# QizhiPei/FABind

Measured on AMD Instinct MI355X. Metric: complexes/sec fwd+bwd (1500p/40l nodes), full IaBNet on the whole graph (pocket model + 4-layer complex model + distance-map head on all nodes / pairs) with the pocket-cls + pocket-centre + coord + distmap + distmap-by-coords + distill losses (BASELINE configs[2] read literally), higher is better.
Workload: dtype bf16

## Files before the change

### fabind_amd/_lib.py

```python
import ctypes
import os

import torch

from . import config as _cfg

_HERE = os.path.dirname(os.path.abspath(__file__))
LIB_PATH = _cfg.knob("FABIND_LIB") or os.path.join(_HERE, "libfabind_hip.so")

ABI_VERSION = 19
DT_F32, DT_BF16 = 0, 1
ACT_NONE, ACT_SILU, ACT_RELU, ACT_SIGMOID, ACT_STORED_DERIV = 0, 1, 2, 3, 4
GEMM_FAM_NT_F32, GEMM_FAM_NT_F32_BF16, GEMM_FAM_NT_BF16, GEMM_FAM_GLDS, GEMM_FAM_PIPE, GEMM_FAM_X3, GEMM_FAM_X3_PRO, GEMM_FAM_PERSIST = range(8)

_vp, _i, _f, _l = ctypes.c_void_p, ctypes.c_int, ctypes.c_float, ctypes.c_long


class GemmArgs(ctypes.Structure):
    _fields_ = [(n, _vp) for n in ("A", "A2", "W", "C", "bias", "R", "r_index", "dotvec", "dot_out", "aux", "groups", "C2")] + \
               [(n, _i) for n in ("M", "N", "K", "K1", "lda", "lda2", "ldw", "ldc", "ldr", "ldaux", "dot_ld",
                                  "a_dtype", "w_dtype", "c_dtype", "aux_dtype", "act_pro", "act_epi", "dact_epi",
                                  "accumulate", "store_preact", "n_groups", "max_m", "max_n", "groups_ext", "epi_fast", "k_splits")] + \
               [("alpha", _f), ("p_drop", _f), ("drop_seed", ctypes.c_uint)] + \
               [(n, _vp) for n in ("row_mu", "row_rs", "col_c", "C16")] + [("ldc16", _i), ("split3", _i), ("r_dtype", _i), ("c2_bf16", _i)]
# ... 105 lines not shown
    "fabind_rowdot_bwd": [_vp, _i, _vp, _i, _vp, _i, _i, _i, _vp, _vp, _vp, _i, _vp],
    "fabind_edge_geom_bwd": [_vp, _vp, _vp, _vp, _vp, _vp, _vp, _vp, _vp, _vp, _i, _i, _i, _vp, _vp, _vp, _vp],
    "fabind_gcl_pre_bwd": [_vp, _i, _i, _vp, _vp, _i, _vp, _vp, _vp, _i, _vp],
    "fabind_gather_dact": [_vp, _i, _vp, _vp, _i, _i, _vp, _i, _i, _i, _vp],
    "fabind_coord_update_bwd": [_vp, _vp, _vp, _i, _i, _f, _vp, _vp, _vp, _vp],
    "fabind_cross_attn_bwd": [_vp, _i, _vp, _i, _vp, _i, _i, _i, _vp, _i, _i, _i, _f, _vp, _vp, _vp, _vp, _vp, _vp, _vp,
                              _vp, _vp, _vp],
    "fabind_pair_bias_cat": [_vp, _i, _vp, _i, _i, _i, _vp, _i, _vp, _i, _vp, _vp, _i, _vp, _i, _vp, _vp],
    "fabind_batched_transpose_pad": [_vp, _i, _vp, _i, _i, _i, _i, _vp, _vp],
    "fabind_node_chain_fwd": [_vp, _i, _vp, _i, _vp, _vp, _vp, _vp, _vp, _vp, _i, _i, _vp, _i, _vp, _i, _vp, _i, _i, _i, _vp],
    "fabind_node_chain_x3_fwd": [_vp, _i, _vp, _i, _vp, _vp, _vp, _vp, _vp, _vp, _vp, _vp, _vp, _vp, _i, _i, _vp, _i, _vp, _i, _vp, _i, _vp, _i, _vp, _i,
                                 _i, _i, _vp],
    "fabind_rows_hadamard_bwd": [_vp, _i, _i, _vp, _i, _i, _vp, _vp, _vp, _i, _vp, _i, _vp],
    "fabind_pair_hadamard_bwd_grid": [_vp, _i, _i, _vp, _i, _i, _vp, _vp, _vp, _vp, _i, _vp, _i, _vp],
    "fabind_pair_hadamard_bwd_rows": [_vp, _i, _i, _vp, _i, _i, _vp, _i, _i, _vp, _vp, _vp, _vp, _i, _vp, _i, _vp, _i, _vp],
    "fabind_pair_hadamard_bwd": [_vp, _i, _i, _vp, _vp, _i, _i, _vp, _vp, _i, _i, _vp, _vp, _i, _vp, _vp, _i, _vp, _vp, _i,
                                 _vp],
    "fabind_inter_attn_bwd": [_vp, _i, _vp, _i, _i, _vp, _vp, _vp, _vp, _vp, _vp, _vp, _vp, _vp, _vp, _vp, _vp, _f, _i,
                              _vp, _vp, _vp, _vp, _vp, _vp, _vp, _vp, _vp, _vp, _i, _vp],
    "fabind_inter_attn_bwd_rows": [_vp, _i, _vp, _i, _i, _vp, _vp, _vp, _vp, _vp, _vp, _vp, _vp, _vp, _vp, _vp, _vp, _f, _i,
                                   _vp, _vp, _vp, _vp, _vp, _vp, _vp, _vp, _vp, _vp, _i, _vp, _i, _i, _vp],
    "fabind_las_step_bwd": [_vp, _vp, _vp, _vp, _vp, _vp, _vp, _vp, _i, _i, _f, _f, _vp, _vp, _vp],
    "fabind_pair_bias_bwd": [_vp, _i, _vp, _i, _i, _vp, _vp, _i, _i, _i, _vp, _vp, _vp, _vp, _vp],
    "fabind_pair_bias_btcat": [_vp, _i, _vp, _vp, _vp, _i, _i, _i, _vp, _i, _i, _vp],
    "fabind_pair_bias_finish": [_vp, _vp, _i, _i, _vp, _vp, _i, _vp, _vp, _l, _vp],
    "fabind_pack_frag_multi": [_vp, _vp, _i, _vp],
    "fabind_lower_bound": [_vp, _i, _vp, _i, _vp, _vp],
    "fabind_pocket_center_fwd": [_vp, _vp, _vp, _vp, _i, _i, _f, _i, _vp, _vp, _vp],
    "fabind_pocket_center_bwd": [_vp, _vp, _vp, _vp, _i, _i, _f, _vp, _vp, _vp, _vp, _vp],
    "fabind_pair_dist_fwd": [_vp, _i, _i, _vp, _vp, _f, _f, _f, _vp, _vp],
    "fabind_pair_dist_bwd": [_vp, _i, _i, _vp, _vp, _vp, _f, _f, _f, _vp, _vp, _vp],
    "fabind_block_hadamard_fwd": [_vp, _i, _i, _vp, _i, _vp, _i, _i, _vp, _i, _vp],
    "fabind_block_hadamard_bwd": [_vp, _i, _i, _vp, _i, _vp, _i, _vp, _i, _i, _vp, _i, _i, _vp, _vp, _i, _vp, _i, _vp],
    "fabind_loss_fwd": [_vp, _vp, _l, _vp, _vp, _vp, _l, _vp, _vp, _i, _vp, _l, _vp, _vp, _l, _f, _f, _f, _f, _f, _f, _vp, _vp, _vp, _vp, _vp, _vp],
    "fabind_loss_bwd": [_vp, _vp, _l, _vp, _vp, _vp, _l, _vp, _vp, _i, _l, _vp, _vp, _l, _f, _f, _f, _f, _f, _f, _vp, _vp, _vp,
                        _vp, _vp, _vp, _vp, _vp, _vp],
    "fabind_layernorm_fwd": [_vp, _vp, _vp, _f, _i, _i, _vp, _vp, _vp, _vp],
    "fabind_layernorm_bwd": [_vp, _vp, _vp, _vp, _vp, _i, _i, _vp, _vp, _vp, _vp],
}

_lib = None


def load():
    global _lib
    if _lib is not None:
        return _lib
    if not os.path.exists(LIB_PATH):
        raise RuntimeError(
            "fabind_amd: %s is missing -- build it with `python -m fabind_amd.build` (hipcc, gfx950). "
            "There is no CPU/eager fallback for the hot path." % LIB_PATH)
    lib = ctypes.CDLL(LIB_PATH)
    lib.fabind_last_error.restype = ctypes.c_char_p
    lib.fabind_abi_version.restype = ctypes.c_int
    got = lib.fabind_abi_version()
    if got != ABI_VERSION:
        raise RuntimeError("fabind_amd: %s has ABI version %d, this binding needs %d -- rebuild with `python -m fabind_amd.build`"
                           % (LIB_PATH, got, ABI_VERSION))
    lib.fabind_sizeof_args.argtypes, lib.fabind_sizeof_args.restype = [ctypes.c_int], ctypes.c_int
    lib.fabind_cross_attn_bwd_scratch.argtypes, lib.fabind_cross_attn_bwd_scratch.restype = [_i, _i, _i], ctypes.c_long
    lib.fabind_pair_bias_cat_parts.argtypes, lib.fabind_pair_bias_cat_parts.restype = [_i, _i], ctypes.c_long
    lib.fabind_cross_attn_fused_bwd_scratch.argtypes, lib.fabind_cross_attn_fused_bwd_scratch.restype = [_i, _i, _i, _i, _i], ctypes.c_long
    lib.fabind_cross_attn_fused_bwd_parts.argtypes, lib.fabind_cross_attn_fused_bwd_parts.restype = [_i, _i], ctypes.c_int
    lib.fabind_pair_bias_finish_parts.argtypes, lib.fabind_pair_bias_finish_parts.restype = [_i], ctypes.c_int
    lib.fabind_loss_blocks.argtypes, lib.fabind_loss_blocks.restype = [_l, _l, _l], ctypes.c_int
    for nm in ("fabind_pair_block_tile", "fabind_pair_block_chunk"):
# ... 58 lines not shown
```

### fabind_amd/build.py

```python
import os
import subprocess
import sys

HERE = os.path.dirname(os.path.abspath(__file__))
CSRC = os.path.join(HERE, "csrc")
INCLUDE = os.path.join(os.path.dirname(HERE), "include")
LIB = os.path.join(HERE, "libfabind_hip.so")
SOURCES = ["capi.hip", "gemm.hip", "graph.hip", "gcl.hip", "fused_edge.hip", "fused_edge_fwd2.hip", "fused_edge_fwd3.hip", "fused_edge_bwd3.hip", "fused_edge_bwd4.hip", "pair_fused.hip", "attn.hip", "inter_attn_rows.hip", "attn_mfma.hip", "norm.hip", "bwd.hip", "post_optim.hip", "node_chain.hip", "heads.hip", "symmetry.hip", "optim.hip", "ranking.hip"]
HIPCC = os.environ.get("HIPCC", "/opt/rocm/bin/hipcc")
FLAGS = ["--offload-arch=gfx950", "-O3", "-std=c++17", "-fPIC", "-Wno-comment", "-I" + INCLUDE, "-I" + CSRC]


def _stale(out, deps):
    if not os.path.exists(out):
        return True
    t = os.path.getmtime(out)
    return any(os.path.getmtime(d) > t for d in deps)


def build(force=False, verbose=True):
    objs = []
    hdrs = [os.path.join(CSRC, "common.h"), os.path.join(CSRC, "fused_common.h"), os.path.join(INCLUDE, "fabind_hip.h")]
    procs = []
    for src in SOURCES:
        sp = os.path.join(CSRC, src)
        if not os.path.exists(sp):
            raise RuntimeError("fabind_amd.build: source %s is missing" % sp)
        obj = os.path.join(CSRC, src.replace(".hip", ".o"))
        objs.append(obj)
        if force or _stale(obj, [sp] + hdrs):
            cmd = [HIPCC] + FLAGS + ["-c", sp, "-o", obj]
            if verbose:
                print(" ".join(cmd), flush=True)
            procs.append((src, subprocess.Popen(cmd)))
    for src, p in procs:
        if p.wait() != 0:
            raise RuntimeError("hipcc failed on " + src)
    if force or procs or _stale(LIB, objs):
        cmd = [HIPCC, "--offload-arch=gfx950", "-shared", "-fPIC", "-o", LIB] + objs
        if verbose:
            print(" ".join(cmd), flush=True)
# ... 7 lines not shown
```

### fabind_amd/models/model.py

```python
import random

import torch
import torch.nn as nn
import torch.nn.functional as F
from torch.nn import Linear

from .. import kernels as K
from .. import ops
from ..utils.utils import get_keepNode_tensor, gumbel_softmax_no_random
from .att_model import EfficientMCAttModel


class Transition_diff_out_dim(nn.Module):

    def __init__(self, embedding_channels=256, out_channels=256, n=4):
        super().__init__()
        self.layernorm = nn.LayerNorm(embedding_channels)
        self.linear1 = Linear(embedding_channels, n * embedding_channels)
        self.linear2 = Linear(n * embedding_channels, out_channels)
        torch.nn.init.xavier_uniform_(self.linear1.weight, gain=0.001)
        torch.nn.init.xavier_uniform_(self.linear2.weight, gain=0.001)

    def forward(self, z):
        shp = z.shape
# ... 252 lines not shown
        start = _offsets(reps)
        j = torch.arange(pi.shape[0], device=dev) - start[pi]
        ci = _offsets(ncnt)[pocket_batch][pi] + j
        kn = torch.stack([kcnt, ncnt]).tolist()
        return _Pairs(pi, ci, ops.PairBlocks(kn[0], kn[1], dev))

    def _complex_and_heads(self, data, g, plan=None):
        scale = self.coordinate_scale
        cb = data['compound'].batch
        if plan:
            Xn, Xl, cidx, pidx = plan['Xn'], plan['Xl'], plan['cidx'], plan['pidx']
        else:
            Xn = self.normalize_coord(g['X'].unsqueeze(-2)).float()
            Xl = self.normalize_coord(g['XL'].unsqueeze(-2)).float()
            seg1 = g['segment'].bool() if not g['segment'].is_floating_point() else g['segment'] > 0.5
            cidx = torch.nonzero(~seg1 & ~g['is_global']).squeeze(1)
            pidx = torch.nonzero(seg1 & ~g['is_global']).squeeze(1)
        Xo, Ho = self.complex_model(Xn, g['H'], batch_id=g['batch'], segment_id=g['segment'], mask=g['mask'],
                                    is_global=g['is_global'], compound_edge_index=g['c2c'], LAS_edge_index=g['LAS'],
                                    batched_complex_coord_LAS=Xl, LAS_mask=None)
        coords_n = ops.take_unique_rows(Xo, cidx).squeeze(-2)
        return Ho, cidx, pidx, coords_n

    def _dist_heads(self, data, g, Ho, cidx, pidx, coords_n):
        cb = data['compound'].batch
        pairs = g.get('pairs')
        if pairs is None:
            B = int(cb[-1].item()) + 1
            pairs = self._pair_lists(g['pocket_batch'], cb, torch.bincount(g['pocket_batch'], minlength=B), torch.bincount(cb, minlength=B))
        pi, ci = pairs
        ln = ops.layernorm(ops.take_unique_rows(Ho, torch.cat([pidx, cidx])), self.layernorm.weight, self.layernorm.bias, self.layernorm.eps)
        npk = pidx.shape[0]
        blocks = getattr(pairs, 'blocks', None)
        hd = ops.rows_hadamard(ln, pi, npk + ci, a_sorted=True, blocks=blocks, n_a=npk)
        wd = ops.mm_dtype()
        part = ops.linear_rowdot(hd, self.distmap_mlp[0].weight.to(wd), self.distmap_mlp[0].bias,
                                 self.distmap_mlp[2].weight[0].contiguous(), act_epi=K.ACT_RELU)
        y_pred = (part.sum(1) + self.distmap_mlp[2].bias).sigmoid() * 10
        xp = self.normalize_coord(g['pocket_xyz']).float()
        if blocks is not None and coords_n.is_cuda:
            y_by = ops.pair_dist(xp, coords_n, blocks, scale=self.coordinate_scale, lo=0.0, hi=10.0)
        else:
            y_by = self.unnormalize_coord((xp[pi] - ops.take_rows_few(coords_n, ci)).norm(dim=-1)).clamp(0, 10)
        return y_pred, y_by

    def forward(self, data, stage=1, train=False, plan=None):
        cb = data['compound'].batch
        if plan is not None:
            self._adopt_plan(plan, cb.device)
        if plan is not None:
            keep_idx = plan['keep_idx']
        else:
            keep_idx = torch.nonzero(data['pocket'].keepNode).squeeze(1) if (stage == 1 or self.pocket_pred_model.training) else None
        head = self._pocket_head(data, plan)
        training = self.pocket_pred_model.training
        center = self._soft_center(head['logits'], head['mask'], head['xyz'], noise=training)
        pocket_cls = torch.zeros_like(head['mask'], dtype=data.pocket_idx.dtype)
        pocket_cls[head['pb'], head['loc']] = data.pocket_idx
        if training:
            dist = torch.norm(data.coords_center - center, p=2, dim=-1).mean(dim=-1)
            final_stage = 2 if (dist < self.args.center_dist_threshold and random.random() < self.stage_prob) else 1
        else:
            final_stage = stage
        if final_stage == 2:
            c2 = center
            if self.args.local_eval or (self.args.train_pred_pocket_noise and train):
                c2 = center + self.args.train_pred_pocket_noise * (2 * torch.rand_like(center) - 1)
            g = self._stage2(data, head, c2)
        else:
            cx = data['complex']
            pemb = ops.take_unique_rows(head['p_out'], keep_idx if keep_idx is not None else torch.nonzero(data['pocket'].keepNode).squeeze(1))
# ... 62 lines not shown
```

### fabind_amd/ops.py

```python
import ctypes

import numpy as np
import torch

from . import config as _cfg
from . import kernels as K
from ._lib import GemmArgs, check, dt_code, load, ptr, stream


def act_dtype():
    return torch.float32 if _cfg.fp32_storage() else torch.bfloat16


mm_dtype = act_dtype


def needs_grad(*ts):
    return torch.is_grad_enabled() and any(torch.is_tensor(t) and t.requires_grad for t in ts)


_needs_grad = needs_grad


def _nchunk(rows):
# ... 1755 lines not shown


def six_term_loss(coords, y_pred, y_by, logits, center, coords_true, dis_map, pocket_cls, p_mask, center_true, w):
    f = lambda t: t.float().contiguous()
    cls = pocket_cls.contiguous()
    if cls.dtype not in _CLS_DT:
        cls = cls.float()
    m8 = p_mask.contiguous().view(torch.uint8) if p_mask.dtype == torch.bool else p_mask.to(torch.uint8).contiguous()
    w = {k: float(v) for k, v in w.items()}
    loss, terms = _SixTermLoss.apply(f(coords), f(y_pred), f(y_by), f(logits), f(center), f(coords_true), f(dis_map), cls, m8,
                                     f(center_true), w)
    tt = terms.unbind(0)
    return loss, {n: tt[i] for i, n in enumerate(LOSS_TERM_NAMES)}


_PAIRBLOCK = np.dtype([("pair_off", np.int64), ("P", np.int32), ("C", np.int32), ("p_row0", np.int32), ("c_row0", np.int32),
                       ("tile0", np.int32), ("pad", np.int32)])


class PairBlocks:

    def __init__(self, kcnt, ncnt, dev):
        from .param_pack import _upload
        kc, nc = np.asarray(kcnt, dtype=np.int64), np.asarray(ncnt, dtype=np.int64)
        B = kc.shape[0]
        tp, ch = load().fabind_pair_block_tile(), load().fabind_pair_block_chunk()
        tiles = (kc + tp - 1) // tp
        d = np.zeros(B, dtype=_PAIRBLOCK)
        d["pair_off"] = np.cumsum(kc * nc) - kc * nc
        d["P"], d["C"] = kc, nc
        d["p_row0"], d["c_row0"] = np.cumsum(kc) - kc, np.cumsum(nc) - nc
        d["tile0"] = np.cumsum(tiles) - tiles
        self.B, self.n_tiles, self.n_pairs = int(B), int(tiles.sum()), int((kc * nc).sum())
        self.max_C, self.n_prows, self.n_crows = int(nc.max()) if B else 0, int(kc.sum()), int(nc.sum())
        self.nchunk_max = (self.max_C + ch - 1) // ch
        self.chunk = ch
        row_b = np.repeat(np.arange(B, dtype=np.int32), nc)
        raw = np.concatenate([d.view(np.uint8), row_b.view(np.uint8)]) if B else np.zeros(0, dtype=np.uint8)
        self.buf = _upload(raw, dev) if raw.shape[0] else None
        self.desc_bytes = d.view(np.uint8).shape[0]

    def tensors(self):
        return [self.buf] if self.buf is not None else []

    @property
    def desc_ptr(self):
        return self.buf.data_ptr()

    @property
    def row_b_ptr(self):
        return self.buf.data_ptr() + self.desc_bytes


class _PairDist(torch.autograd.Function):
    @staticmethod
    def forward(ctx, xp, xc, blocks, scale, lo, hi):
        y = torch.empty(blocks.n_pairs, dtype=torch.float32, device=xc.device)
        check(load().fabind_pair_dist_fwd(blocks.desc_ptr, blocks.B, blocks.n_tiles, ptr(xp), ptr(xc), scale, lo, hi, ptr(y), stream()),
              "fabind_pair_dist_fwd")
        ctx.save_for_backward(xp, xc)
        ctx.blocks, ctx.k = blocks, (scale, lo, hi)
        return y

    @staticmethod
    def backward(ctx, dy):
        xp, xc = ctx.saved_tensors
        bl = ctx.blocks
        part = torch.empty((bl.B, 8, bl.max_C, 3), dtype=torch.float32, device=xc.device)
        dxc = torch.empty_like(xc)
        check(load().fabind_pair_dist_bwd(bl.desc_ptr, bl.B, bl.max_C, ptr(xp), ptr(xc), ptr(dy.contiguous().float()), ctx.k[0], ctx.k[1],
                                          ctx.k[2], ptr(part), ptr(dxc), stream()), "fabind_pair_dist_bwd")
        return None, dxc, None, None, None, None


def pair_dist(xp, xc, blocks, scale=1.0, lo=0.0, hi=10.0):
    assert not xp.requires_grad, "pair_dist: the pocket coordinates are data"
    xp, xc = xp.float().contiguous(), xc.float().contiguous()
    assert xp.shape[0] == blocks.n_prows and xc.shape[0] == blocks.n_crows
    return _PairDist.apply(xp, xc, blocks, float(scale), float(lo), float(hi))


RANK_MODES = {"logsigmoid": 0, "dynamic_hinge": 1}
RANK_MAX_GROUP = 1024
COUNT_NAMES = ("ranked_right", "pairs", "hit", "confidence_correct")
# ... 74 lines not shown
```

### include/fabind_hip.h

```cpp
#ifndef FABIND_HIP_H
#define FABIND_HIP_H

#include <stdint.h>

#ifdef __cplusplus
extern "C" {
#endif

#ifndef __HIP_PLATFORM_AMD__
typedef struct ihipStream_t* hipStream_t;
#endif

const char* fabind_last_error(void);
#define FABIND_ABI_VERSION 19
int fabind_abi_version(void);
int fabind_sizeof_args(int which);

typedef struct FabindGemmArgs {
    const void* A;
    const void* A2;
    const void* W;
    void* C;
    const float* bias;
    const void* R;
// ... 243 lines not shown
int fabind_las_step(const float* x, const float* x0, const int* las_i, const int* las_j, const int* las_off,
                    const int* node_off, const int* c_cnt, int B, int max_n, float step, float clampv, float* x_out,
                    unsigned char* pass_mask, hipStream_t stream);

int fabind_pocket_center_fwd(const float* logits, const uint8_t* mask, const float* xyz, const float* noise, int B, int L,
                             float tau, int hard, float* center, float* wsum, hipStream_t stream);
int fabind_pocket_center_bwd(const float* logits, const uint8_t* mask, const float* xyz, const float* noise, int B, int L,
                             float tau, const float* center, const float* wsum, const float* dcenter, float* dlogits,
                             hipStream_t stream);

int fabind_loss_blocks(long n_pair, long n_coord, long n_cls);
int fabind_loss_fwd(const float* coords, const float* coords_true, long n_coord, const float* y_pred, const float* y_by,
                    const float* dis_map, long n_pair, const float* logits, const void* cls, int cls_dt, const uint8_t* mask,
                    long n_cls, const float* center, const float* center_true, long n_center, float w_coord, float w_pair,
                    float w_distill, float w_cls, float w_center, float delta, float* part, unsigned* ticket, float* out,
                    float* loss_out, float* terms_out, hipStream_t stream);
int fabind_loss_bwd(const float* coords, const float* coords_true, long n_coord, const float* y_pred, const float* y_by,
                    const float* dis_map, long n_pair, const float* logits, const void* cls, int cls_dt, long n_cls,
                    const float* center, const float* center_true, long n_center, float w_coord, float w_pair, float w_distill,
                    float w_cls, float w_center, float delta, const float* fwd_out, const float* g_loss, const float* g_terms,
                    float* d_coords, float* d_y_pred, float* d_y_by, float* d_logits, float* d_center, hipStream_t stream);

int fabind_pair_block_tile(void);
int fabind_pair_block_chunk(void);
int fabind_pair_dist_fwd(const void* desc, int B, int n_tiles, const float* xp, const float* xc, float scale, float lo, float hi,
                         float* y, hipStream_t stream);
int fabind_pair_dist_bwd(const void* desc, int B, int max_C, const float* xp, const float* xc, const float* dy, float scale, float lo,
                         float hi, float* part, float* dxc, hipStream_t stream);
int fabind_block_hadamard_fwd(const void* desc, int B, int n_tiles, const float* tp, int ldtp, const float* tc, int ldtc, int W, void* out,
                              int ldo, hipStream_t stream);
int fabind_block_hadamard_bwd(const void* desc, int B, int n_tiles, const void* dout, int ldo, const float* tp, int ldtp,
                              const float* tc, int ldtc, int W, const int* row_b, int n_crows, int nchunk_max, float* part,
                              float* dtp, int lddp, float* dtc, int lddc, hipStream_t stream);

int fabind_select_rows(const float* x, const float* z, const uint8_t* mask, int n, int width, float* x_out,
                       hipStream_t stream);

int fabind_row_stats(const void* x, int x_dt, int ldx, float eps, int R, int C, float* mu, float* rs, hipStream_t stream);

int fabind_layernorm_rows(const void* x, int x_dt, int ldx, const float* w, const float* b, float eps, int R, int C, void* y,
                          int y_dt, int ldy, int pad_to, hipStream_t stream);
int fabind_edge_ln_concat(const float* h, int ldh, int H, const int* row, const int* col, const float* rhohat, const float* w,
                          const float* b, float eps, int E, void* y, int y_dt, int ldy, int pad_to, hipStream_t stream);

int fabind_edge_lnfold(const void* AB, int ldab, int Kp, int H, const int* row, const int* col, const float* rho,
                       const float* stat, float eps, const float* w_r, const float* c_r, const float* c_c, const float* dvec,
                       int E, void* out, float p_drop, unsigned seed, hipStream_t stream);
int fabind_edge_lnfold_bwd_blocks(int E);
int fabind_edge_lnfold_bwd(const void* AB, int ldab, int Kp, int H, const int* row, const int* col, const float* rho,
                           const float* stat, float eps, const float* w_r, const float* c_r, const float* c_c,
                           const void* out, const void* dout, int E, float p_drop, void* du, float* es,
                           float* drho, float* part, int n_blocks, hipStream_t stream);

int fabind_inter_coord_fold(const void* P, int ldp, int H, const int* col, const float* rho, const float* stat, float q_w,
                            float eps, const float* u, const float* d, const float* w3, int E, float* s_out, float p_drop,
                            unsigned seed, hipStream_t stream);
int fabind_layernorm_rows_bwd(const void* x, int x_dt, int ldx, const float* w, const void* dy, int dy_dt, int lddy, float eps,
                              int R, int C, void* dx, int dx_dt, int lddx, float* dw_part, float* db_part, int nblk, hipStream_t stream);
int fabind_edge_concat(const float* h, int ldh, int H, const int* row, const int* col, const float* rhohat, int E, void* y,
                       int y_dt, int ldy, int pad_to, hipStream_t stream);
int fabind_layernorm_fwd(const float* x, const float* w, const float* b, float eps, int R, int C, float* y, float* mean,
                         float* rstd, hipStream_t stream);
int fabind_layernorm_bwd(const float* x, const float* w, const float* dy, const float* mean, const float* rstd, int R,
                         int C, float* dx, float* dw_part, float* db_part, hipStream_t stream);

int fabind_add(const float* a, const float* b, float* out, long n, hipStream_t stream);
// ... 93 lines not shown
```

Measured before the change: 529.6.

## Fuse distance-map head hadamard, linear, ReLU and row-dot into persistent HIP kernels

Adds a dedicated persistent kernel for the distance-map head forward. Per pair tile it gathers the pocket and ligand rows, forms their elementwise product into LDS, runs the 512x512 MFMA GEMM, and applies bias, ReLU and the dot with the output weight in the epilogue. It stores the pre-activation as bf16 for backward. A fused backward kernel computes the masked upstream gradient, the bias and u column reductions and the input-gradient GEMM in one pass, then reuses the existing block-hadamard backward. This is meant to remove separate hadamard and GEMM launches and the extra traffic of the intermediate between them, at the cost of extra bf16 scratch buffers and a path that only supports H=512 in bf16.

```diff
diff --git a/fabind_amd/_lib.py b/fabind_amd/_lib.py
--- a/fabind_amd/_lib.py
+++ b/fabind_amd/_lib.py
@@ -161,6 +161,8 @@
     "fabind_pair_dist_bwd": [_vp, _i, _i, _vp, _vp, _vp, _f, _f, _f, _vp, _vp, _vp],
     "fabind_block_hadamard_fwd": [_vp, _i, _i, _vp, _i, _vp, _i, _i, _vp, _i, _vp],
     "fabind_block_hadamard_bwd": [_vp, _i, _i, _vp, _i, _vp, _i, _vp, _i, _i, _vp, _i, _i, _vp, _vp, _i, _vp, _i, _vp],
+    "fabind_dist_head_fwd": [_vp, _i, _l, _vp, _i, _i, _vp, _i, _i, _i, _vp, _vp, _vp, _vp, _vp, _vp, _i, _vp],
+    "fabind_dist_head_bwd": [_l, _vp, _vp, _vp, _i, _vp, _vp, _vp, _vp, _i, _vp],
     "fabind_loss_fwd": [_vp, _vp, _l, _vp, _vp, _vp, _l, _vp, _vp, _i, _vp, _l, _vp, _vp, _l, _f, _f, _f, _f, _f, _f, _vp, _vp, _vp, _vp, _vp, _vp],
     "fabind_loss_bwd": [_vp, _vp, _l, _vp, _vp, _vp, _l, _vp, _vp, _i, _l, _vp, _vp, _l, _f, _f, _f, _f, _f, _f, _vp, _vp, _vp,
                         _vp, _vp, _vp, _vp, _vp, _vp],
diff --git a/fabind_amd/build.py b/fabind_amd/build.py
--- a/fabind_amd/build.py
+++ b/fabind_amd/build.py
@@ -6,7 +6,7 @@
 CSRC = os.path.join(HERE, "csrc")
 INCLUDE = os.path.join(os.path.dirname(HERE), "include")
 LIB = os.path.join(HERE, "libfabind_hip.so")
-SOURCES = ["capi.hip", "gemm.hip", "graph.hip", "gcl.hip", "fused_edge.hip", "fused_edge_fwd2.hip", "fused_edge_fwd3.hip", "fused_edge_bwd3.hip", "fused_edge_bwd4.hip", "pair_fused.hip", "attn.hip", "inter_attn_rows.hip", "attn_mfma.hip", "norm.hip", "bwd.hip", "post_optim.hip", "node_chain.hip", "heads.hip", "symmetry.hip", "optim.hip", "ranking.hip"]
+SOURCES = ["capi.hip", "gemm.hip", "graph.hip", "gcl.hip", "fused_edge.hip", "fused_edge_fwd2.hip", "fused_edge_fwd3.hip", "fused_edge_bwd3.hip", "fused_edge_bwd4.hip", "pair_fused.hip", "attn.hip", "inter_attn_rows.hip", "attn_mfma.hip", "norm.hip", "bwd.hip", "post_optim.hip", "node_chain.hip", "heads.hip", "dist_head.hip", "symmetry.hip", "optim.hip", "ranking.hip"]
 HIPCC = os.environ.get("HIPCC", "/opt/rocm/bin/hipcc")
 FLAGS = ["--offload-arch=gfx950", "-O3", "-std=c++17", "-fPIC", "-Wno-comment", "-I" + INCLUDE, "-I" + CSRC]
 
diff --git a/fabind_amd/csrc/dist_head.hip b/fabind_amd/csrc/dist_head.hip
--- /dev/null
+++ b/fabind_amd/csrc/dist_head.hip
@@ -0,0 +1,354 @@
+#include "common.h"
+#include "fabind_hip.h"
+#include "fused_common.h"
+
+namespace {
+
+struct PairBlock { long pair_off; int P, C, p_row0, c_row0, tile0, pad; };
+static_assert(sizeof(PairBlock) == 32, "PairBlock is the 32-byte record of include/fabind_hip.h");
+
+__device__ __forceinline__ int dh_find(const PairBlock* __restrict__ desc, int B, long g) {
+    int lo = 0, hi = B - 1;
+    while (lo < hi) {
+        const int mid = (lo + hi + 1) >> 1;
+        if (desc[mid].pair_off <= g) lo = mid; else hi = mid - 1;
+    }
+    return lo;
+}
+
+typedef unsigned dh_u32x2_t __attribute__((ext_vector_type(2)));
+__device__ __forceinline__ void dh_stq(bf16_t* p_, uint32_t a, uint32_t b) { __builtin_nontemporal_store(dh_u32x2_t{a, b}, (dh_u32x2_t*)p_); }
+__device__ __forceinline__ uint2 dh_ldq(const bf16_t* p_) { const dh_u32x2_t v = __builtin_nontemporal_load((const dh_u32x2_t*)p_); return make_uint2(v.x, v.y); }
+__device__ __forceinline__ fe_f2 dh_relu(const fe_f2 z) { return fe_f2{fmaxf(z.x, 0.f), fmaxf(z.y, 0.f)}; }
+
+#define DH_OPAQUE(v_) asm volatile("" : "+v"(v_))
+#define DH_QOFF(i, j) (lb_ + (i) * 16 * H + ((cx_ ^ ((j) * 2)) * 8))
+#define DH_FOFF(i, j) (fbase + (size_t)((i) * 4 + (j)) * 256)
+
+template <int H>
+__global__ __launch_bounds__(H, 4) void dist_head_fwd_kernel(const PairBlock* __restrict__ desc, int B, long n_pairs,
+                                                             const float* __restrict__ tp, int ldtp, unsigned tp_bytes,
+                                                             const float* __restrict__ tc, int ldtc, unsigned tc_bytes,
+                                                             const bf16_t* __restrict__ W1p, const float* __restrict__ b1,
+                                                             const float* __restrict__ u, bf16_t* __restrict__ hd,
+                                                             bf16_t* __restrict__ zf, float* __restrict__ part) {
+    constexpr int BM = FE_BM, MI = BM / 16;
+    constexpr int NW = H / 64;
+    constexpr int CH = H / 8;
+    constexpr int NIT = BM / NW;
+    constexpr int PB = 4;
+    constexpr int SWZ = 15;
+    static_assert(CH == 64 && NIT % PB == 0, "one 16-byte chunk per lane: H = 512");
+    extern __shared__ __attribute__((aligned(16))) unsigned char smem[];
+    bf16_t* sX = (bf16_t*)smem;
+    int* sTab = (int*)(sX + BM * H);
+    float* sDot = (float*)(sTab + 4 * BM);
+    const int tid = threadIdx.x, lane = tid & 63, wave = tid >> 6;
+    const int fr = lane & 15, cq = lane >> 4;
+    const int n_tiles = (int)((n_pairs + BM - 1) / BM);
+    const __amdgpu_buffer_rsrc_t rs_tp = fe_rsrc(const_cast<float*>(tp), tp_bytes);
+    const __amdgpu_buffer_rsrc_t rs_tc = fe_rsrc(const_cast<float*>(tc), tc_bytes);
+    const int cx = (wave * 8 + (cq >> 1)) ^ (fr & SWZ);
+    const int lbase = fr * H + (cq & 1) * 4;
+    const int fcol = wave * 64 + cq * 4;
+
+    int tb_p = -1, tb_c = -1;
+    auto fetch_tables = [&](int tile) {
+        if (tid < BM) {
+            const long g = (long)tile * BM + tid;
+            tb_p = -1; tb_c = -1;
+            if (g < n_pairs) {
+                const PairBlock d = desc[dh_find(desc, B, g)];
+                const long l = g - d.pair_off;
+                const int C = max(d.C, 1);
+                const int i = (int)(l / C);
+                tb_p = d.p_row0 + i;
+                tb_c = d.c_row0 + (int)(l - (long)i * C);
+            }
+        }
+    };
+    auto commit_tables = [&](int hb) {
+        if (tid < BM) { sTab[hb * 2 * BM + tid] = tb_p; sTab[hb * 2 * BM + BM + tid] = tb_c; }
+    };
+    fetch_tables(blockIdx.x);
+    commit_tables(0);
+    __syncthreads();
+    int hb = 0;
+
+    for (int tile = blockIdx.x; tile < n_tiles; tile += gridDim.x, hb ^= 1) {
+        const long e0 = (long)tile * BM;
+        const long rem = n_pairs - e0;
+        const int ne = rem < BM ? (int)rem : BM;
+        const int* sP = sTab + hb * 2 * BM;
+        const int* sC = sP + BM;
+        int lz = 0;
+        asm volatile("" : "+s"(lz));
+        const bf16_t* Wp = W1p + lz;
+        const float* b1_ = b1 + lz;
+        const float* u_ = u + lz;
+
+        {
+            int ch_ = lane, rw_ = wave;
+            DH_OPAQUE(ch_); DH_OPAQUE(rw_);
+            const __amdgpu_buffer_rsrc_t rs_hd = fe_rsrc(hd + (size_t)e0 * H, (unsigned)ne * H * 2);
+#pragma unroll
+            for (int u0 = 0; u0 < NIT; u0 += PB) {
+                uint4 pa[PB][2], qa[PB][2];
+#pragma unroll
+                for (int v = 0; v < PB; ++v) {
+                    const int e = (u0 + v) * NW + rw_;
+                    const unsigned po = ((unsigned)max(sP[e], 0) * (unsigned)ldtp + ch_ * 8) * 4;
+                    const unsigned qo = ((unsigned)max(sC[e], 0) * (unsigned)ldtc + ch_ * 8) * 4;
+                    pa[v][0] = fe3_bload16(rs_tp, po, 0); pa[v][1] = fe3_bload16(rs_tp, po, 16);
+                    qa[v][0] = fe3_bload16(rs_tc, qo, 0); qa[v][1] = fe3_bload16(rs_tc, qo, 16);
+                }
+#pragma unroll
+                for (int v = 0; v < PB; ++v) {
+                    const int e = (u0 + v) * NW + rw_;
+                    const uint4 p0 = pa[v][0], p1 = pa[v][1], q0 = qa[v][0], q1 = qa[v][1];
+#define DH_F(x_) __uint_as_float(x_)
+                    uint4 o = make_uint4(pack2_bf16(DH_F(p0.x) * DH_F(q0.x), DH_F(p0.y) * DH_F(q0.y)), pack2_bf16(DH_F(p0.z) * DH_F(q0.z), DH_F(p0.w) * DH_F(q0.w)),
+                                         pack2_bf16(DH_F(p1.x) * DH_F(q1.x), DH_F(p1.y) * DH_F(q1.y)), pack2_bf16(DH_F(p1.z) * DH_F(q1.z), DH_F(p1.w) * DH_F(q1.w)));
+#undef DH_F
+                    if (e >= ne) o = make_uint4(0u, 0u, 0u, 0u);
+                    *(uint4*)&sX[e * H + ((ch_ ^ (e & SWZ)) * 8)] = o;
+                    __builtin_amdgcn_raw_buffer_store_b128(fe_u32x4_t{o.x, o.y, o.z, o.w}, rs_hd, (int)((e * H + ch_ * 8) * 2), 0,  2);
+                }
+            }
+        }
+        __syncthreads();
+
+        f32x4_t acc[MI][4];
+        fe_zero(acc);
+        fe_gemm_rolled<H, MI, true, SWZ>(sX, Wp, wave, lane, acc);
+
+        const bool has_next = tile + (int)gridDim.x < n_tiles;
+        {
+            int ln_ = lane;
+            DH_OPAQUE(ln_);
+            const size_t fbase = (((size_t)tile * NW + wave) * (MI * 4) * 64 + ln_) * 4;
+            fe_f2 da[MI], db[MI];
+#pragma unroll
+            for (int i = 0; i < MI; ++i) { da[i] = fe_f2{0.f, 0.f}; db[i] = da[i]; }
+#pragma unroll
+            for (int j = 0; j < 4; ++j) {
+                const float4 bq = *(const float4*)(b1_ + fcol + j * 16), wq = *(const float4*)(u_ + fcol + j * 16);
+                const fe_f2 b01 = fe_f2{bq.x, bq.y}, b23 = fe_f2{bq.z, bq.w}, w01 = fe_f2{wq.x, wq.y}, w23 = fe_f2{wq.z, wq.w};
+#pragma unroll
+                for (int i = 0; i < MI; ++i) {
+                    const fe_f2 z01 = fe_f2{acc[i][j][0], acc[i][j][1]} + b01, z23 = fe_f2{acc[i][j][2], acc[i][j][3]} + b23;
+                    da[i] += dh_relu(z01) * w01;
+                    db[i] += dh_relu(z23) * w23;
+                    dh_stq(&zf[DH_FOFF(i, j)], fe3_pack(z01), fe3_pack(z23));
+                }
+                __builtin_amdgcn_sched_barrier(0);
+            }
+            if (has_next) fetch_tables(tile + gridDim.x);
+#pragma unroll
+            for (int i = 0; i < MI; ++i) {
+                float t = (da[i].x + da[i].y) + (db[i].x + db[i].y);
+                t += __shfl_xor(t, 16, 64);
+                t += __shfl_xor(t, 32, 64);
+                if (cq == 0) sDot[wave * BM + i * 16 + fr] = t;
+            }
+        }
+        if (has_next) commit_tables(hb ^ 1);
+        __syncthreads();
+        if (tid < ne) {
+            float s = 0.f;
+#pragma unroll
+            for (int w = 0; w < NW; ++w) s += sDot[w * BM + tid];
+            part[e0 + tid] = s;
+        }
+    }
+}
+
+template <int H>
+__global__ __launch_bounds__(H, 4) void dist_head_bwd_kernel(long n_pairs, const bf16_t* __restrict__ zf, const float* __restrict__ dpart,
+                                                             const float* __restrict__ u, const bf16_t* __restrict__ W1Tp,
+                                                             bf16_t* __restrict__ dz, bf16_t* __restrict__ dhd, float* __restrict__ part) {
+    constexpr int BM = FE_BM, MI = BM / 16;
+    constexpr int NW = H / 64;
+    constexpr int CH = H / 8;
+    constexpr int SWZ = 15;
+    static_assert(BM <= H, "one thread per table row");
+    extern __shared__ __attribute__((aligned(16))) unsigned char smem[];
+    bf16_t* sX = (bf16_t*)smem;
+    float* sTab = (float*)(sX + BM * H);
+    float* sPart = sTab + 2 * BM;
+    const int tid = threadIdx.x, lane = tid & 63, wave = tid >> 6;
+    const int fr = lane & 15, cq = lane >> 4;
+    const int n_tiles = (int)((n_pairs + BM - 1) / BM);
+    const int cx = (wave * 8 + (cq >> 1)) ^ (fr & SWZ);
+    const int lbase = fr * H + (cq & 1) * 4;
+    const int fcol = wave * 64 + cq * 4;
+    sPart[tid] = 0.f; sPart[H + tid] = 0.f;
+
+    float tb_d = 0.f;
+    auto fetch_tables = [&](int tile) {
+        if (tid < BM) {
+            const long g = (long)tile * BM + tid;
+            tb_d = g < n_pairs ? dpart[g] : 0.f;
+        }
+    };
+    auto commit_tables = [&](int hb) { if (tid < BM) sTab[hb * BM + tid] = tb_d; };
+    fetch_tables(blockIdx.x);
+    commit_tables(0);
+    __syncthreads();
+    int hb = 0;
+
+    for (int tile = blockIdx.x; tile < n_tiles; tile += gridDim.x, hb ^= 1) {
+        const long e0 = (long)tile * BM;
+        const long rem = n_pairs - e0;
+        const int ne = rem < BM ? (int)rem : BM;
+        const float* sDp = sTab + hb * BM;
+        int lz = 0;
+        asm volatile("" : "+s"(lz));
+        const float* u_ = u + lz;
+        const bf16_t* Wp = W1Tp + lz;
+        auto copy_out = [&](bf16_t* dst) {
+            const __amdgpu_buffer_rsrc_t rs = fe_rsrc(dst + (size_t)e0 * H, (unsigned)ne * H * 2);
+            int t_ = tid;
+            DH_OPAQUE(t_);
+#pragma unroll
+            for (int it = 0; it < BM * CH / H; ++it) {
+                const int q = t_ + it * H;
+                const int rw = q / CH, c8 = q % CH;
+                const uint4 v = *(const uint4*)&sX[rw * H + ((c8 ^ (rw & SWZ)) * 8)];
+                __builtin_amdgcn_raw_buffer_store_b128(fe_u32x4_t{v.x, v.y, v.z, v.w}, rs, (int)((rw * H + c8 * 8) * 2), 0,  2);
+            }
+        };
+        const bool has_next = tile + (int)gridDim.x < n_tiles;
+        if (has_next) fetch_tables(tile + gridDim.x);
+
+        {
+            int cx_ = cx, lb_ = lbase, ln_ = lane;
+            DH_OPAQUE(cx_); DH_OPAQUE(lb_); DH_OPAQUE(ln_);
+            const size_t fbase = (((size_t)tile * NW + wave) * (MI * 4) * 64 + ln_) * 4;
+            uint2 zq[4][MI];
+#pragma unroll
+            for (int j = 0; j < 4; ++j)
+#pragma unroll
+                for (int i = 0; i < MI; ++i) zq[j][i] = dh_ldq(&zf[DH_FOFF(i, j)]);
+            float dsr[MI];
+#pragma unroll
+            for (int i = 0; i < MI; ++i) dsr[i] = sDp[i * 16 + fr];
+            float4 wq4[4];
+#pragma unroll
+            for (int j = 0; j < 4; ++j) wq4[j] = *(const float4*)(u_ + fcol + j * 16);
+#pragma unroll
+            for (int j = 0; j < 4; ++j) {
+                const fe_f2 w01 = fe_f2{wq4[j].x, wq4[j].y}, w23 = fe_f2{wq4[j].z, wq4[j].w};
+                fe_f2 aua = fe_f2{0.f, 0.f}, aub = aua, aba = aua, abb = aua;
+#pragma unroll
+                for (int i = 0; i < MI; ++i) {
+                    const fe_f2 z01 = fe3_unpack(zq[j][i].x), z23 = fe3_unpack(zq[j][i].y);
+                    const fe_f2 g01 = w01 * dsr[i], g23 = w23 * dsr[i];
+                    const fe_f2 t01 = fe_f2{z01.x > 0.f ? g01.x : 0.f, z01.y > 0.f ? g01.y : 0.f};
+                    const fe_f2 t23 = fe_f2{z23.x > 0.f ? g23.x : 0.f, z23.y > 0.f ? g23.y : 0.f};
+                    const uint32_t k01 = fe3_pack(t01), k23 = fe3_pack(t23);
+                    aua += dh_relu(z01) * dsr[i]; aub += dh_relu(z23) * dsr[i];
+                    aba += fe3_unpack(k01); abb += fe3_unpack(k23);
+                    *(uint2*)&sX[DH_QOFF(i, j)] = make_uint2(k01, k23);
+                }
+                float au[4] = {aua.x, aua.y, aub.x, aub.y}, ab[4] = {aba.x, aba.y, abb.x, abb.y};
+#pragma unroll
+                for (int r = 0; r < 4; ++r) { au[r] = fe3_row16_sum(au[r]); ab[r] = fe3_row16_sum(ab[r]); }
+                if (fr < 4) {
+                    const float vb = fr == 0 ? ab[0] : fr == 1 ? ab[1] : fr == 2 ? ab[2] : ab[3];
+                    const float vu = fr == 0 ? au[0] : fr == 1 ? au[1] : fr == 2 ? au[2] : au[3];
+                    sPart[fcol + j * 16 + fr] += vb;
+                    sPart[H + fcol + j * 16 + fr] += vu;
+                }
+                __builtin_amdgcn_sched_barrier(0);
+            }
+        }
+        __syncthreads();
+
+        copy_out(dz);
+        f32x4_t acc[MI][4];
+        fe_zero(acc);
+        fe_gemm_rolled<H, MI, true, SWZ>(sX, Wp, wave, lane, acc);
+        __syncthreads();
+
+        {
+            int cx_ = cx, lb_ = lbase;
+            DH_OPAQUE(cx_); DH_OPAQUE(lb_);
+#pragma unroll
+            for (int j = 0; j < 4; ++j)
+#pragma unroll
+                for (int i = 0; i < MI; ++i)
+                    *(uint2*)&sX[DH_QOFF(i, j)] = make_uint2(pack2_bf16(acc[i][j][0], acc[i][j][1]), pack2_bf16(acc[i][j][2], acc[i][j][3]));
+        }
+        if (has_next) commit_tables(hb ^ 1);
+        __syncthreads();
+        copy_out(dhd);
+        __syncthreads();
+    }
+    __syncthreads();
+    float* po = part + (size_t)blockIdx.x * 2 * H;
+    po[tid] = sPart[tid];
+    po[H + tid] = sPart[H + tid];
+}
+
+#undef DH_OPAQUE
+#undef DH_QOFF
+#undef DH_FOFF
+
+template <typename KernelT>
+int dh_set_lds(KernelT k, size_t lds) {
+    const hipError_t e = hipFuncSetAttribute((const void*)k, hipFuncAttributeMaxDynamicSharedMemorySize, (int)lds);
+    if (e != hipSuccess) { fabind_set_error(hipGetErrorString(e)); return (int)e; }
+    return 0;
+}
+
+}
+
+extern "C" int fabind_dist_head_fwd(const void* desc, int B, long n_pairs, const float* tp, int ldtp, int n_prows, const float* tc, int ldtc,
+                                    int n_crows, int H, const void* W1p, const float* b1, const float* u, void* hd, void* zf, float* part,
+                                    int n_groups, hipStream_t stream) {
+    FB_REQUIRE(H == 512, "fabind_dist_head_fwd: H = 512 only");
+    if (n_pairs <= 0) return 0;
+    FB_REQUIRE(desc && B > 0 && tp && tc && W1p && b1 && u && hd && zf && part && n_groups > 0, "fabind_dist_head_fwd: null operand / scratch");
+    FB_REQUIRE(ldtp >= H && ldtc >= H && ldtp % 4 == 0 && ldtc % 4 == 0 &&
+                   ((((uintptr_t)tp | (uintptr_t)tc | (uintptr_t)W1p | (uintptr_t)b1 | (uintptr_t)u | (uintptr_t)hd | (uintptr_t)zf) & 15) == 0),
+               "fabind_dist_head_fwd: 16-byte aligned rows");
+    FB_REQUIRE(n_prows > 0 && n_crows > 0 && (size_t)n_prows * ldtp * 4 < (1ull << 32) && (size_t)n_crows * ldtc * 4 < (1ull << 32),
+               "fabind_dist_head_fwd: the pocket / ligand operands are addressed with 32-bit byte offsets");
+    const long n_tiles = (n_pairs + FE_BM - 1) / FE_BM;
+    FB_REQUIRE(n_tiles < (1l << 30), "fabind_dist_head_fwd: too many pairs");
+    const size_t lds = (size_t)FE_BM * H * 2 + (size_t)4 * FE_BM * sizeof(int) + (size_t)(H / 64) * FE_BM * sizeof(float);
+    static bool set_ = false;
+    if (!set_) {
+        if (const int rc = dh_set_lds(dist_head_fwd_kernel<512>, lds)) return rc;
+        set_ = true;
+    }
+    const unsigned tp_bytes = (unsigned)(((size_t)(n_prows - 1) * ldtp + H) * 4), tc_bytes = (unsigned)(((size_t)(n_crows - 1) * ldtc + H) * 4);
+    const int ng = (int)(n_groups < n_tiles ? n_groups : n_tiles);
+    hipLaunchKernelGGL((dist_head_fwd_kernel<512>), dim3(ng), dim3(512), lds, stream, (const PairBlock*)desc, B, n_pairs, tp, ldtp, tp_bytes,
+                       tc, ldtc, tc_bytes, (const bf16_t*)W1p, b1, u, (bf16_t*)hd, (bf16_t*)zf, part);
+    FB_CHECK_LAUNCH();
+    return 0;
+}
+
+extern "C" int fabind_dist_head_bwd(long n_pairs, const void* zf, const float* dpart, const float* u, int H, const void* W1Tp, void* dz,
+                                    void* dhd, float* part, int n_groups, hipStream_t stream) {
+    FB_REQUIRE(H == 512, "fabind_dist_head_bwd: H = 512 only");
+    FB_REQUIRE(part && n_groups > 0, "fabind_dist_head_bwd: part (n_groups x 2 x H floats of scratch) is required");
+    const long n_tiles = (n_pairs + FE_BM - 1) / FE_BM;
+    FB_REQUIRE(n_pairs > 0 && n_groups <= n_tiles, "fabind_dist_head_bwd: 1 <= n_groups <= ceil(n_pairs / 64) (every work-group writes its partials)");
+    FB_REQUIRE(zf && dpart && u && W1Tp && dz && dhd, "fabind_dist_head_bwd: null operand");
+    FB_REQUIRE(((((uintptr_t)zf | (uintptr_t)u | (uintptr_t)W1Tp | (uintptr_t)dz | (uintptr_t)dhd) & 15) == 0) && (((uintptr_t)dpart & 3) == 0),
+               "fabind_dist_head_bwd: 16-byte aligned rows");
+    FB_REQUIRE(n_tiles < (1l << 30), "fabind_dist_head_bwd: too many pairs");
+    const size_t lds = (size_t)FE_BM * H * 2 + (size_t)2 * FE_BM * sizeof(float) + (size_t)2 * H * sizeof(float);
+    static bool set_ = false;
+    if (!set_) {
+        if (const int rc = dh_set_lds(dist_head_bwd_kernel<512>, lds)) return rc;
+        set_ = true;
+    }
+    hipLaunchKernelGGL((dist_head_bwd_kernel<512>), dim3(n_groups), dim3(512), lds, stream, n_pairs, (const bf16_t*)zf, dpart, u,
+                       (const bf16_t*)W1Tp, (bf16_t*)dz, (bf16_t*)dhd, part);
+    FB_CHECK_LAUNCH();
+    return 0;
+}
diff --git a/fabind_amd/models/model.py b/fabind_amd/models/model.py
--- a/fabind_amd/models/model.py
+++ b/fabind_amd/models/model.py
@@ -308,11 +308,13 @@
         ln = ops.layernorm(ops.take_unique_rows(Ho, torch.cat([pidx, cidx])), self.layernorm.weight, self.layernorm.bias, self.layernorm.eps)
         npk = pidx.shape[0]
         blocks = getattr(pairs, 'blocks', None)
-        hd = ops.rows_hadamard(ln, pi, npk + ci, a_sorted=True, blocks=blocks, n_a=npk)
-        wd = ops.mm_dtype()
-        part = ops.linear_rowdot(hd, self.distmap_mlp[0].weight.to(wd), self.distmap_mlp[0].bias,
-                                 self.distmap_mlp[2].weight[0].contiguous(), act_epi=K.ACT_RELU)
-        y_pred = (part.sum(1) + self.distmap_mlp[2].bias).sigmoid() * 10
+        W1, b1, u = self.distmap_mlp[0].weight, self.distmap_mlp[0].bias, self.distmap_mlp[2].weight[0].contiguous()
+        if ops.dist_head_fused_ok(ln, blocks, npk, W1, b1, u):
+            part = ops.dist_head(ln, blocks, npk, W1, b1, u)
+        else:
+            hd = ops.rows_hadamard(ln, pi, npk + ci, a_sorted=True, blocks=blocks, n_a=npk)
+            part = ops.linear_rowdot(hd, W1.to(ops.mm_dtype()), b1, u, act_epi=K.ACT_RELU).sum(1)
+        y_pred = (part + self.distmap_mlp[2].bias).sigmoid() * 10
         xp = self.normalize_coord(g['pocket_xyz']).float()
         if blocks is not None and coords_n.is_cuda:
             y_by = ops.pair_dist(xp, coords_n, blocks, scale=self.coordinate_scale, lo=0.0, hi=10.0)
diff --git a/fabind_amd/ops.py b/fabind_amd/ops.py
--- a/fabind_amd/ops.py
+++ b/fabind_amd/ops.py
@@ -1811,6 +1811,7 @@
         d["p_row0"], d["c_row0"] = np.cumsum(kc) - kc, np.cumsum(nc) - nc
         d["tile0"] = np.cumsum(tiles) - tiles
         self.B, self.n_tiles, self.n_pairs = int(B), int(tiles.sum()), int((kc * nc).sum())
+        self._kc, self._nc = kc, nc
         self.max_C, self.n_prows, self.n_crows = int(nc.max()) if B else 0, int(kc.sum()), int(nc.sum())
         self.nchunk_max = (self.max_C + ch - 1) // ch
         self.chunk = ch
@@ -1822,6 +1823,14 @@
     def tensors(self):
         return [self.buf] if self.buf is not None else []
 
+    def pair_lists(self):
+        kc, nc = self._kc, self._nc
+        p0, c0 = np.cumsum(kc) - kc, np.cumsum(nc) - nc
+        pi = np.concatenate([np.repeat(np.arange(p, p + k), n) for p, k, n in zip(p0, kc, nc)] or [np.zeros(0, np.int64)])
+        ci = np.concatenate([np.tile(np.arange(c, c + n), k) for c, k, n in zip(c0, kc, nc)] or [np.zeros(0, np.int64)])
+        dev = self.buf.device if self.buf is not None else "cpu"
+        return torch.from_numpy(pi.astype(np.int64)).to(dev), torch.from_numpy(ci.astype(np.int64)).to(dev)
+
     @property
     def desc_ptr(self):
         return self.buf.data_ptr()
@@ -1829,6 +1838,100 @@
     @property
     def row_b_ptr(self):
         return self.buf.data_ptr() + self.desc_bytes
+
+
+DIST_HEAD_FUSED = True
+
+
+_DH_FRAGS = {}
+
+
+def _dist_head_frags(W):
+    import weakref
+    key = (W._version, W.data_ptr(), W.device)
+    c = _DH_FRAGS.get(id(W))
+    if c is not None and c[0]() is W and c[1] == key:
+        return c[2]
+    with torch.no_grad():
+        Wd = W.detach().to(torch.bfloat16)
+        packs = tuple(K.pack_frag_multi([Wd, Wd.t()]))
+    _DH_FRAGS[id(W)] = (weakref.ref(W, lambda _r, k=id(W): _DH_FRAGS.pop(k, None)), key, packs)
+    return packs
+
+
+def _dist_head_groups(dev, n_pairs):
+    ng = K._N_CU.get(dev)
+    if ng is None:
+        ng = K._N_CU[dev] = torch.cuda.get_device_properties(dev).multi_processor_count
+    return max(1, min(2 * ng, (n_pairs + 63) // 64))
+
+
+def dist_head_fused_ok(t, blocks, n_a, W1, b1, u):
+    return bool(DIST_HEAD_FUSED and blocks is not None and _cfg.get_precision() == "bf16" and act_dtype() == torch.bfloat16 and t.is_cuda
+                and t.dim() == 2 and t.shape[1] == 512 and tuple(W1.shape) == (512, 512) and t.dtype == torch.float32 and t.stride(1) == 1
+                and t.stride(0) % 4 == 0 and t.data_ptr() % 16 == 0 and n_a == blocks.n_prows and t.shape[0] == blocks.n_prows + blocks.n_crows
+                and blocks.n_pairs > 0 and blocks.n_prows > 0 and blocks.n_crows > 0 and t.shape[0] * t.stride(0) * 4 < 2 ** 32
+                and b1 is not None and b1.dtype == torch.float32 and u.dtype == torch.float32 and u.shape == (512,)
+                and _needs_grad(t, W1, b1, u))
+
+
+class _DistHead(torch.autograd.Function):
+
+    @staticmethod
+    def forward(ctx, t, W, b, u, blocks, n_a, frags):
+        bl, dev, H = blocks, t.device, 512
+        n = bl.n_pairs
+        n_tiles = (n + 63) // 64
+        b, u = b.contiguous(), u.contiguous()
+        hd = torch.empty((n, H), dtype=torch.bfloat16, device=dev)
+        zf = torch.empty((n_tiles * 64, H), dtype=torch.bfloat16, device=dev)
+        part = torch.empty(n, dtype=torch.float32, device=dev)
+        K._profiled("dist_head_fwd_kernel<512> pairs=%d" % n, 2.0 * n * H * H,
+                    lambda: check(load().fabind_dist_head_fwd(bl.desc_ptr, bl.B, n, ptr(t), t.stride(0), bl.n_prows, ptr(t[n_a:]), t.stride(0), bl.n_crows,
+                                                              H, ptr(frags[0]), ptr(b), ptr(u), ptr(hd), ptr(zf), ptr(part),
+                                                              _dist_head_groups(dev, n), stream()), "fabind_dist_head_fwd"),
+                    4.0 * n * H)
+        ctx.blocks, ctx.n_a, ctx.frags = bl, n_a, frags
+        ctx.save_for_backward(t, W, u, hd, zf)
+        return part
+
+    @staticmethod
+    def backward(ctx, dpart):
+        t, W, u, hd, zf = ctx.saved_tensors
+        bl, n_a, H, dev = ctx.blocks, ctx.n_a, 512, t.device
+        n = bl.n_pairs
+        dpart = dpart.contiguous().float()
+        ng = _dist_head_groups(dev, n)
+        dz = torch.empty((n, H), dtype=torch.bfloat16, device=dev)
+        dhd = torch.empty((n, H), dtype=torch.bfloat16, device=dev)
+        cols = torch.empty((ng, 2, H), dtype=torch.float32, device=dev)
+        K._profiled("dist_head_bwd_kernel<512> pairs=%d" % n, 2.0 * n * H * H,
+                    lambda: check(load().fabind_dist_head_bwd(n, ptr(zf), ptr(dpart), ptr(u), H, ptr(ctx.frags[1]), ptr(dz), ptr(dhd), ptr(cols), ng,
+                                                              stream()), "fabind_dist_head_bwd"),
+                    6.0 * n * H)
+        ni = ctx.needs_input_grad
+        dt_ = None
+        if ni[0]:
+            dt_ = torch.empty_like(t)
+            hp = torch.empty((bl.n_tiles, bl.nchunk_max, bl.chunk, H), dtype=torch.float32, device=dev)
+            tc, dtc = t[n_a:], dt_[n_a:]
+            check(load().fabind_block_hadamard_bwd(bl.desc_ptr, bl.B, bl.n_tiles, ptr(dhd), H, ptr(t), t.stride(0), ptr(tc), t.stride(0), H,
+                                                   bl.row_b_ptr, bl.n_crows, bl.nchunk_max, ptr(hp), ptr(dt_), dt_.stride(0), ptr(dtc),
+                                                   dt_.stride(0), stream()), "fabind_block_hadamard_bwd")
+        ps = cols.sum(0)
+        dW, db = _param_grads(dz, hd, None, W, ni[1], ni[2], db=ps[0])
+        return dt_, dW, db, (ps[1] if ni[3] else None), None, None, None
+
+
+def dist_head(t, blocks, n_a, W1, b1, u):
+    if dist_head_fused_ok(t, blocks, n_a, W1, b1, u):
+        frags = _dist_head_frags(W1)
+        W = W1.to(mm_dtype())
+        K.tn_hook(W, b1)
+        return _DistHead.apply(t, W, b1, u, blocks, n_a, frags)
+    pi, ci = blocks.pair_lists()
+    hd = rows_hadamard(t, pi, n_a + ci, a_sorted=True, blocks=blocks, n_a=n_a)
+    return linear_rowdot(hd, W1.to(mm_dtype()), b1, u, act_epi=K.ACT_RELU).sum(1)
 
 
 class _PairDist(torch.autograd.Function):
diff --git a/include/fabind_hip.h b/include/fabind_hip.h
--- a/include/fabind_hip.h
+++ b/include/fabind_hip.h
@@ -299,6 +299,12 @@
 int fabind_block_hadamard_bwd(const void* desc, int B, int n_tiles, const void* dout, int ldo, const float* tp, int ldtp,
                               const float* tc, int ldtc, int W, const int* row_b, int n_crows, int nchunk_max, float* part,
                               float* dtp, int lddp, float* dtc, int lddc, hipStream_t stream);
+
+int fabind_dist_head_fwd(const void* desc, int B, long n_pairs, const float* tp, int ldtp, int n_prows, const float* tc, int ldtc,
+                         int n_crows, int H, const void* W1p, const float* b1, const float* u, void* hd, void* zf, float* part,
+                         int n_groups, hipStream_t stream);
+int fabind_dist_head_bwd(long n_pairs, const void* zf, const float* dpart, const float* u, int H, const void* W1Tp, void* dz, void* dhd,
+                         float* part, int n_groups, hipStream_t stream);
 
 int fabind_select_rows(const float* x, const float* z, const uint8_t* mask, int n, int width, float* x_out,
                        hipStream_t stream);
```

Result: no change. 540.5, median of 6 (+2.1%).
